# RViMLab/ECCV2022-multi-scale-and-cross-scale-contrastive-segmentation

Hardware: NVIDIA B200
Metric: ms+cs contrastive loss fwd+bwd anchor-pairs/s (higher is better)
Workload: dtype bf16

## Files before the change

eccv2022-multi-scale-and-cross-scale-contrastive-segmentation_b200/csrc/common.cuh:

```cuda
#pragma once
#include <cuda_runtime.h>
#include <cuda_bf16.h>
#include <cuda_fp16.h>
#include <stdint.h>
#include <stdio.h>
#include <stdarg.h>

#include "../../include/mscs.h"

namespace mscs {

void set_error(const char* fmt, ...);
const char* get_error();

#define MSCS_CHECK_ARG(cond, ...)                                   \
  do {                                                              \
    if (!(cond)) { ::mscs::set_error(__VA_ARGS__); return -1; }     \
  } while (0)

#define MSCS_CUDA(expr)                                                                   \
  do {                                                                                    \
    cudaError_t _e = (expr);                                                              \
    if (_e != cudaSuccess) {                                                              \
      ::mscs::set_error("%s failed: %s (%s:%d)", #expr, cudaGetErrorString(_e), __FILE__, \
                        __LINE__);                                                        \
      return (int)_e;                                                                     \
    }                                                                                     \
  } while (0)

#define MSCS_LAUNCH_CHECK()                                                               \
  do {                                                                                    \
    cudaError_t _e = cudaGetLastError();                                                  \
    if (_e != cudaSuccess) {                                                              \
      ::mscs::set_error("kernel launch failed: %s (%s:%d)", cudaGetErrorString(_e),       \
                        __FILE__, __LINE__);                                              \
      return (int)_e;                                                                     \
    }                                                                                     \
  } while (0)

static inline size_t align_up(size_t v, size_t a) { return (v + a - 1) / a * a; }
static inline int ceil_div(int a, int b) { return (a + b - 1) / b; }

bool pdl_enabled();

__device__ __forceinline__ void pdl_trigger() { asm volatile("griddepcontrol.launch_dependents;" ::: "memory"); }
__device__ __forceinline__ void pdl_wait() { asm volatile("griddepcontrol.wait;" ::: "memory"); }

template <typename... P, typename... A>
static inline cudaError_t launch_k(void (*kernel)(P...), dim3 grid, dim3 block, size_t smem, cudaStream_t st, A&&... args) {
  cudaLaunchConfig_t cfg{};
  cfg.gridDim = grid; cfg.blockDim = block; cfg.dynamicSmemBytes = smem; cfg.stream = st;
  cudaLaunchAttribute at{};
  at.id = cudaLaunchAttributeProgrammaticStreamSerialization;
  at.val.programmaticStreamSerializationAllowed = 1;
  cfg.attrs = &at;
  cfg.numAttrs = pdl_enabled() ? 1 : 0;
  return cudaLaunchKernelEx(&cfg, kernel, static_cast<P>(args)...);
}

__device__ __forceinline__ float warp_sum(float v) {
#pragma unroll
  for (int o = 16; o > 0; o >>= 1) v += __shfl_xor_sync(0xffffffffu, v, o);
  return v;
}

__device__ __forceinline__ float to_f32(float x) { return x; }
__device__ __forceinline__ float to_f32(__nv_bfloat16 x) { return __bfloat162float(x); }
__device__ __forceinline__ float to_f32(__half x) { return __half2float(x); }
template <typename T> __device__ __forceinline__ T from_f32(float x);
template <> __device__ __forceinline__ float from_f32<float>(float x) { return x; }
template <> __device__ __forceinline__ __nv_bfloat16 from_f32<__nv_bfloat16>(float x) { return __float2bfloat16_rn(x); }
template <> __device__ __forceinline__ __half from_f32<__half>(float x) { return __float2half_rn(x); }

__device__ __forceinline__ uint32_t pack2(__nv_bfloat16*, float a, float b) {
  const __nv_bfloat162 h = __floats2bfloat162_rn(a, b);
  return reinterpret_cast<const uint32_t&>(h);
}
__device__ __forceinline__ uint32_t pack2(__half*, float a, float b) {
  const __half2 h = __floats2half2_rn(a, b);
  return reinterpret_cast<const uint32_t&>(h);
}

__device__ __forceinline__ void st16_cs(float* p, const float (&v)[4]) {
  __stcs(reinterpret_cast<float4*>(p), make_float4(v[0], v[1], v[2], v[3]));
}
template <typename T>
__device__ __forceinline__ void st16_cs(T* p, const float (&v)[8]) {
  const uint4 u = make_uint4(pack2(p, v[0], v[1]), pack2(p, v[2], v[3]), pack2(p, v[4], v[5]), pack2(p, v[6], v[7]));
  __stcs(reinterpret_cast<uint4*>(p), u);
}

__device__ __forceinline__ void ld4(const float* p, float (&v)[4]) {
  const float4 x = *reinterpret_cast<const float4*>(p);
  v[0] = x.x; v[1] = x.y; v[2] = x.z; v[3] = x.w;
}
template <typename T>
__device__ __forceinline__ void ld4(const T* p, float (&v)[4]) {
  const uint2 u = *reinterpret_cast<const uint2*>(p);
  const T* h = reinterpret_cast<const T*>(&u);
#pragma unroll
  for (int q = 0; q < 4; ++q) v[q] = to_f32(h[q]);
}
__device__ __forceinline__ void st4_cs(float* p, const float (&v)[4]) { st16_cs(p, v); }
template <typename T>
__device__ __forceinline__ void st4_cs(T* p, const float (&v)[4]) {
  __stcs(reinterpret_cast<uint2*>(p), make_uint2(pack2(p, v[0], v[1]), pack2(p, v[2], v[3])));
}

static inline int dtype_bytes(int dtype) {
  return dtype == MSCS_DTYPE_F32 ? 4 : (dtype == MSCS_DTYPE_BF16 || dtype == MSCS_DTYPE_F16) ? 2 : 0;
}
// ... 3 lines not shown
```

eccv2022-multi-scale-and-cross-scale-contrastive-segmentation_b200/csrc/ptx.cuh:

```cuda
#pragma once
#include <cuda.h>
#include <cuda_runtime.h>
#include <stdint.h>

namespace mscs {
namespace ptx {

__device__ __forceinline__ uint32_t smem_u32(const void* p) {
  return static_cast<uint32_t>(__cvta_generic_to_shared(p));
}

__device__ __forceinline__ bool elect_one() {
  uint32_t pred;
  asm volatile(
      "{\n\t.reg .pred P;\n\t"
      "elect.sync _|P, 0xffffffff;\n\t"
      "selp.b32 %0, 1, 0, P;\n\t}"
      : "=r"(pred));
  return pred != 0;
}

__device__ __forceinline__ void mbar_init(uint64_t* bar, uint32_t count) {
  asm volatile("mbarrier.init.shared::cta.b64 [%0], %1;" ::"r"(smem_u32(bar)), "r"(count) : "memory");
}
// ... 179 lines not shown
  d |= (uint64_t)((sbo_bytes >> 4) & 0x3FFFu) << 32;
  d |= (uint64_t)1 << 46;
  d |= (uint64_t)2 << 61;
  return d;
}
__host__ __device__ constexpr uint32_t umma_idesc_bf16(int M, int N, int a_mn_major, int b_mn_major) {
  return (1u << 4) | (1u << 7) | (1u << 10) | ((uint32_t)a_mn_major << 15) | ((uint32_t)b_mn_major << 16) |
         ((uint32_t)(N >> 3) << 17) | ((uint32_t)(M >> 4) << 24);
}
__device__ __forceinline__ void umma_ss(uint32_t d_tmem, uint64_t a_desc, uint64_t b_desc, uint32_t idesc,
                                        uint32_t accumulate) {
  asm volatile(
      "{\n\t.reg .pred p;\n\t"
      "setp.ne.b32 p, %4, 0;\n\t"
      "tcgen05.mma.cta_group::1.kind::f16 [%0], %1, %2, %3, p;\n\t}"
      ::"r"(d_tmem), "l"(a_desc), "l"(b_desc), "r"(idesc), "r"(accumulate)
      : "memory");
}
__device__ __forceinline__ void umma_ts(uint32_t d_tmem, uint32_t a_tmem, uint64_t b_desc, uint32_t idesc,
                                        uint32_t accumulate) {
  asm volatile(
      "{\n\t.reg .pred p;\n\t"
      "setp.ne.b32 p, %4, 0;\n\t"
      "tcgen05.mma.cta_group::1.kind::f16 [%0], [%1], %2, %3, p;\n\t}"
      ::"r"(d_tmem), "r"(a_tmem), "l"(b_desc), "r"(idesc), "r"(accumulate)
      : "memory");
}
__device__ __forceinline__ void umma_ts2(uint32_t d_tmem, uint32_t a_tmem, uint32_t b_lo, uint32_t b_hi, uint32_t idesc,
                                         uint32_t accumulate) {
  asm volatile(
      "{\n\t.reg .pred p;\n\t.reg .b64 bd;\n\t"
      "setp.ne.b32 p, %5, 0;\n\t"
      "mov.b64 bd, {%2, %3};\n\t"
      "tcgen05.mma.cta_group::1.kind::f16 [%0], [%1], bd, %4, p;\n\t}"
      ::"r"(d_tmem), "r"(a_tmem), "r"(b_lo), "r"(b_hi), "r"(idesc), "r"(accumulate)
      : "memory");
}
__device__ __forceinline__ void umma_ss2(uint32_t d_tmem, uint32_t a_lo, uint32_t a_hi, uint32_t b_lo, uint32_t b_hi,
                                         uint32_t idesc, uint32_t accumulate) {
  asm volatile(
      "{\n\t.reg .pred p;\n\t.reg .b64 ad, bd;\n\t"
      "setp.ne.b32 p, %6, 0;\n\t"
      "mov.b64 ad, {%1, %2};\n\t"
      "mov.b64 bd, {%3, %4};\n\t"
      "tcgen05.mma.cta_group::1.kind::f16 [%0], ad, bd, %5, p;\n\t}"
      ::"r"(d_tmem), "r"(a_lo), "r"(a_hi), "r"(b_lo), "r"(b_hi), "r"(idesc), "r"(accumulate)
      : "memory");
}
__device__ __forceinline__ void umma_commit(uint64_t* bar) {
  asm volatile("tcgen05.commit.cta_group::1.mbarrier::arrive::one.shared::cluster.b64 [%0];" ::"r"(smem_u32(bar))
               : "memory");
}

__device__ __forceinline__ float ex2(float x) {
  float y;
  asm("ex2.approx.ftz.f32 %0, %1;" : "=f"(y) : "f"(x));
  return y;
}
__device__ __forceinline__ float ex2_poly(float v, float scale) {
  const float magic = 12582912.f;
  const float t = fmaf(v, scale, magic);
  const float n = t - magic;
  const float f = fmaf(v, scale, -n);
  float p = fmaf(0.009570100344717503f, f, 0.05591785907745361f);
  p = fmaf(p, f, 0.240247443318367f);
  p = fmaf(p, f, 0.6931217908859253f);
  p = fmaf(p, f, 0.9999992847442627f);
  return __int_as_float(__float_as_int(p) + (__float_as_int(t) << 23));
}
__device__ __forceinline__ uint64_t pack2(float lo, float hi) {
  uint64_t r;
  asm("mov.b64 %0, {%1, %2};" : "=l"(r) : "f"(lo), "f"(hi));
  return r;
}
__device__ __forceinline__ uint64_t pack2u(uint32_t lo, uint32_t hi) {
  uint64_t r;
  asm("mov.b64 %0, {%1, %2};" : "=l"(r) : "r"(lo), "r"(hi));
  return r;
}
__device__ __forceinline__ void unpack2(uint64_t v, float& lo, float& hi) {
  asm("mov.b64 {%0, %1}, %2;" : "=f"(lo), "=f"(hi) : "l"(v));
}
__device__ __forceinline__ uint64_t fma2(uint64_t a, uint64_t b, uint64_t c) {
  uint64_t d;
  asm("fma.rn.f32x2 %0, %1, %2, %3;" : "=l"(d) : "l"(a), "l"(b), "l"(c));
  return d;
}
__device__ __forceinline__ uint64_t mul2(uint64_t a, uint64_t b) {
  uint64_t d;
  asm("mul.rn.f32x2 %0, %1, %2;" : "=l"(d) : "l"(a), "l"(b));
  return d;
}
__device__ __forceinline__ uint64_t add2(uint64_t a, uint64_t b) {
  uint64_t d;
  asm("add.rn.f32x2 %0, %1, %2;" : "=l"(d) : "l"(a), "l"(b));
  return d;
}
__device__ __forceinline__ uint64_t ex2_poly2(uint64_t v, uint64_t scale2) {
  const uint64_t magic = pack2(12582912.f, 12582912.f), nmagic = pack2(-12582912.f, -12582912.f);
  const uint64_t t = fma2(v, scale2, magic);
  const uint64_t n = add2(t, nmagic);
  const uint64_t nn = n ^ 0x8000000080000000ull;
  const uint64_t f = fma2(v, scale2, nn);
  uint64_t p = fma2(pack2(0.009570100344717503f, 0.009570100344717503f), f, pack2(0.05591785907745361f, 0.05591785907745361f));
  p = fma2(p, f, pack2(0.240247443318367f, 0.240247443318367f));
  p = fma2(p, f, pack2(0.6931217908859253f, 0.6931217908859253f));
// ... 18 lines not shown
```

eccv2022-multi-scale-and-cross-scale-contrastive-segmentation_b200/csrc/sim_bwd.cu:

```cuda
#include "sim_tc.cuh"
#include <stdlib.h>

namespace mscs {

constexpr int kBwdEpiWarps = 16;
constexpr int kBwdThreads = 128 + 32 * kBwdEpiWarps;
constexpr int kBwdStages = 3;
constexpr int kBwdSub = 64;
constexpr uint32_t kTmX = 256, kTmS = 384;

struct BwdDev {
  const int* row_cls; const int* col_seg;
  const float* row_cs; const float* row_cpn; const float* row_neg;
  const float* col_cs; const float* col_cpn; const float* col_neg;
  const __nv_bfloat16* x_rows;
  float* dF; int ld;
  int n_rows, n_cols, self_mask, y_map;
  float scale_log2, out_scale;
};
struct BwdArgs {
  alignas(64) CUtensorMap maps[MSCS_MAX_SCALES];
  BwdDev p[MSCS_MAX_PASSES];
  WorkTable work;
  const float* grad_out;
  const int* rows_dev[MSCS_MAX_PASSES]; const int* cols_dev[MSCS_MAX_PASSES];
};

__host__ __device__ constexpr size_t bwd_smem_bytes(int KB) {
  return 1024 + (size_t)(kBwdStages * KB) * kBlkBytes + (size_t)kBwdEpiWarps * 2 * 3 * 32 * sizeof(float) + 256;
}

__device__ __forceinline__ uint32_t pack_bf16(float lo, float hi) {
  __nv_bfloat162 v = __floats2bfloat162_rn(lo, hi);
  return *reinterpret_cast<uint32_t*>(&v);
}
__device__ __forceinline__ void red_add_v4(float* addr, float a, float b, float c, float d) {
  asm volatile("red.global.add.v4.f32 [%0], {%1, %2, %3, %4};" ::"l"(addr), "f"(a), "f"(b), "f"(c), "f"(d)
               : "memory");
}

template <int KB, bool DEV>
__global__ void __launch_bounds__(kBwdThreads, 1) k_sim_bwd(const __grid_constant__ BwdArgs args) {
  constexpr int CP = KB * 64;
  extern __shared__ uint8_t smem_raw[];
  uint8_t* smem = reinterpret_cast<uint8_t*>((reinterpret_cast<uintptr_t>(smem_raw) + 1023) & ~uintptr_t(1023));
  uint8_t* smB = smem;
  float* cstat = reinterpret_cast<float*>(smB + (size_t)kBwdStages * KB * kBlkBytes);
  uint64_t* bars = reinterpret_cast<uint64_t*>(cstat + kBwdEpiWarps * 2 * 3 * 32);
  uint64_t* b_full = bars;
  uint64_t* b_empty = bars + 12;
  uint64_t* s_full = bars + 15;
  uint64_t* w_full = bars + 17;
  uint64_t* df_full = bars + 19;  uint64_t* df_empty = bars + 20;
  uint64_t* x_full = bars + 21;
  uint32_t* tmem_slot = reinterpret_cast<uint32_t*>(bars + 22);

  const int warp = threadIdx.x >> 5, lane = threadIdx.x & 31;
  pdl_trigger();
  if (warp == 0 && lane == 0) {
    for (int i = 0; i < kBwdStages; ++i) {
      ptx::mbar_init(&b_full[i], 1);
      ptx::mbar_init(&b_empty[i], 1);
    }
    for (int i = 0; i < 2; ++i) { ptx::mbar_init(&s_full[i], 1); ptx::mbar_init(&w_full[i], kBwdEpiWarps); }
    ptx::mbar_init(df_full, 1); ptx::mbar_init(df_empty, kBwdEpiWarps);
    ptx::mbar_init(x_full, kBwdEpiWarps);
    ptx::fence_barrier_init();
  }
  if (warp == 2) ptx::tmem_alloc(tmem_slot, 512);
  ptx::tc_fence_before();
  __syncthreads();
  ptx::tc_fence_after();
  const uint32_t tmem_base = *tmem_slot;
  pdl_wait();
#if defined(MSCS_WAIT_PROFILE) || defined(MSCS_TRACE)
  const unsigned long long prof_t0 = ptx::globaltimer_ns();
  const long long prof_c0 = clock64();
  (void)prof_t0;
// ... 214 lines not shown
          if (lane == 0) ptx::mbar_arrive(&w_full[sb]);
          MSCS_TRACE_EV(1 + ((warp - 4) >> 3), (warp - 4) & 7, t2);
        }
        publish_cols((un & 1) ^ 1);
      }
      if (warp == 4) MSCS_TRACE_EV(3, 0, 64u + seg);
      if (have_n && cq < KB)
        asm volatile("prefetch.global.L2 [%0];" ::"l"(args.p[nx.owner].x_rows + (size_t)(nx.rb * 128 + r_loc) * CP + cq * 64));
      ptx::mbar_wait(df_full, seg & 1, 222);
      ptx::tc_fence_after();
      if (warp == 4) MSCS_TRACE_EV(3, 1, 64u + seg);
      const float sc = p.out_scale * gout;
      float* drow = p.dF + (size_t)row * p.ld;
#pragma unroll 1
      for (int c0 = cq * (CP / 4); c0 < (cq + 1) * (CP / 4); c0 += 16) {
        uint32_t uu[16];
        ptx::tmem_ld16(tmem_dF + lane_base + c0, uu);
        ptx::tmem_ld_wait16(uu);
        if (valid) {
#pragma unroll
          for (int c = 0; c < 16; c += 4)
            red_add_v4(drow + c0 + c, __uint_as_float(uu[c]) * sc, __uint_as_float(uu[c + 1]) * sc,
                       __uint_as_float(uu[c + 2]) * sc, __uint_as_float(uu[c + 3]) * sc);
        }
      }
      ptx::tc_fence_before();
      __syncwarp();
      if (lane == 0) ptx::mbar_arrive(df_empty);
      if (warp == 4) MSCS_TRACE_EV(3, 2, 64u + seg);
      ++seg;
      sg = nx; have = have_n;
    }
  }
  __syncwarp();
  ptx::tc_fence_before();
  __syncthreads();
  if (warp == 2) ptx::tmem_dealloc(tmem_base, 512);
#ifdef MSCS_TRACE
  if (blockIdx.x == 5 && threadIdx.x == 0) ptx::g_trace[3 * 2048 + 255 * 8 + 6] = (unsigned long long)clock64();
  if (threadIdx.x == 0 && blockIdx.x < 256) {
    ptx::g_trace[3 * 2048 + 1024 + blockIdx.x] = (unsigned long long)(clock64() - prof_c0);
    ptx::g_trace[3 * 2048 + 1280 + blockIdx.x] = prof_t0;
    ptx::g_trace[3 * 2048 + 1536 + blockIdx.x] = ptx::globaltimer_ns();
  }
#endif
#ifdef MSCS_WAIT_PROFILE
  if (blockIdx.x == 0 && threadIdx.x == 0) {
    atomicAdd(&ptx::g_wait_ns[31], ptx::globaltimer_ns() - prof_t0);
    atomicAdd(&ptx::g_wait_cnt[31], (unsigned long long)(clock64() - prof_c0));
  }
#endif
}

}

using namespace mscs;

template <int KB, bool DEV>
static int launch_bwd(const BwdArgs& args, cudaStream_t st) {
  const size_t smem = bwd_smem_bytes(KB);
  if (int rc = ensure_trap_buffer()) return rc;
  MSCS_CUDA(cudaFuncSetAttribute(k_sim_bwd<KB, DEV>, cudaFuncAttributeMaxDynamicSharedMemorySize, (int)smem));
  MSCS_CUDA(launch_k(k_sim_bwd<KB, DEV>, persistent_ctas(), kBwdThreads, smem, st, args));
  MSCS_LAUNCH_CHECK();
  return 0;
}

extern "C" int mscs_sim_backward(const mscs_sim_job* job, const float* grad_out, float* const* dF_sets,
                                 const int32_t* dF_ld, void* stream_) {
  return mscs_sim_backward_sets(job, grad_out, dF_sets, dF_ld, 0xffffffffu, stream_);
}

extern "C" int mscs_sim_backward_sets(const mscs_sim_job* job, const float* grad_out, float* const* dF_sets,
                                      const int32_t* dF_ld, uint32_t set_mask, void* stream_) {
  int rc = validate_job(job);
  if (rc) return rc;
  MSCS_CHECK_ARG(job->work && grad_out && dF_sets && dF_ld, "null pointer argument");
  const bool dev_counts = job->terms[0].n1_dev != nullptr;
  for (int t = 0; t < job->num_terms; ++t)
    MSCS_CHECK_ARG((job->terms[t].n1_dev != nullptr) == dev_counts && (job->terms[t].n2_dev != nullptr) == dev_counts,
                   "term %d: n1_dev / n2_dev must be set for every term or for none", t);
  cudaStream_t st = (cudaStream_t)stream_;
  BwdPass passes[MSCS_MAX_PASSES];
  int np = build_passes(job, passes);
  {
    int kept = 0;
    for (int i = 0; i < np; ++i)
      if ((set_mask >> passes[i].row_set) & 1u) passes[kept++] = passes[i];
    np = kept;
    if (np == 0) return 0;
  }
  size_t fwd_items = 0, ranges = 0;
  for (int t = 0; t < job->num_terms; ++t) {
    fwd_items += (size_t)ceil_div(job->terms[t].N2, 256);
    ranges += align_up(sizeof(int2) * (size_t)job->terms[t].N1, 64) +
              align_up(sizeof(int2) * (size_t)ceil_div(job->terms[t].N1, 128) * 4, 64);
  }
  char* w = (char*)job->work + 4096 + ranges +
            2 * (align_up(sizeof(WorkItem) * fwd_items, 64) + align_up(sizeof(int) * (fwd_items + 1), 64));
  BwdArgs args{};
  args.grad_out = grad_out;
  const void* bases[MSCS_MAX_SCALES]; int nmaps = 0;
  auto map_of = [&](const void* base, int rows) -> int {
    for (int i = 0; i < nmaps; ++i) if (bases[i] == base) return i;
    if (nmaps == MSCS_MAX_SCALES) return -1;
    if (make_tensor_map(&args.maps[nmaps], base, (rows + 255) / 256 * 256, job->C_pad)) return -2;
    bases[nmaps] = base;
    return nmaps++;
  };
  BuildArgs b{};
  int nitems = 0;
  for (int i = 0; i < np; ++i) {
    const BwdPass& p = passes[i];
    const int ym = map_of(p.y_bf16, p.n_cols);
    if (ym == -2) return -1;
    MSCS_CHECK_ARG(ym >= 0, "too many distinct operand matrices");
    MSCS_CHECK_ARG(dF_sets[p.row_set] && dF_ld[p.row_set] >= job->C_pad && dF_ld[p.row_set] % 4 == 0,
                   "pass %d: dF buffer of set %d missing or leading dimension < C_pad", i, p.row_set);
    args.p[i] = BwdDev{p.row_cls, p.col_seg, p.row_cs, p.row_cpn, p.row_neg, p.col_cs, p.col_cpn, p.col_neg,
                       (const __nv_bfloat16*)p.x_bf16, dF_sets[p.row_set], dF_ld[p.row_set], p.n_rows, p.n_cols,
                       p.self_mask, ym, p.scale_log2, p.out_scale};
    b.t[i] = BuildTerm{p.row_cls, p.col_seg, p.n_rows, p.n_cols, nitems, p.rb_lo, 0, 1 << 30, p.n_rows_dev, p.n_cols_dev};
    args.rows_dev[i] = p.n_rows_dev; args.cols_dev[i] = p.n_cols_dev;
    nitems += p.rb_hi - p.rb_lo;
  }
  b.num_terms = np; b.nitems = nitems; b.rows_per_item = 128; b.mode = 0;
  b.pad = 6;
  static const int pad_env = [] { const char* e = getenv("MSCS_BWD_PAD"); return e ? atoi(e) : -1; }();
  if (pad_env >= 0) b.pad = pad_env;
  b.items = (WorkItem*)w; w += align_up(sizeof(WorkItem) * (size_t)nitems, 64);
  b.prefix = (int*)w;
  rc = launch_build_work(b, st);
  if (rc) return rc;
  args.work = WorkTable{b.items, b.prefix, nitems, b.pad};
  if (dev_counts) {
    switch (job->C_pad / 64) {
      case 1: return launch_bwd<1, true>(args, st);
      case 2: return launch_bwd<2, true>(args, st);
      case 3: return launch_bwd<3, true>(args, st);
      default: return launch_bwd<4, true>(args, st);
    }
  }
  switch (job->C_pad / 64) {
    case 1: return launch_bwd<1, false>(args, st);
    case 2: return launch_bwd<2, false>(args, st);
    case 3: return launch_bwd<3, false>(args, st);
    default: return launch_bwd<4, false>(args, st);
  }
}

extern "C" int mscs_debug_wait_profile_bwd(unsigned long long* ns_out, unsigned long long* cnt_out) {
  MSCS_CUDA(cudaDeviceSynchronize());
  MSCS_CUDA(cudaMemcpyFromSymbol(ns_out, ptx::g_wait_ns, sizeof(unsigned long long) * 32));
  MSCS_CUDA(cudaMemcpyFromSymbol(cnt_out, ptx::g_wait_cnt, sizeof(unsigned long long) * 32));
  unsigned long long zero[32] = {};
  MSCS_CUDA(cudaMemcpyToSymbol(ptx::g_wait_ns, zero, sizeof(zero)));
  MSCS_CUDA(cudaMemcpyToSymbol(ptx::g_wait_cnt, zero, sizeof(zero)));
  return 0;
}

extern "C" int mscs_debug_trace_bwd(unsigned long long* out, int max_events) {
#ifdef MSCS_TRACE
  MSCS_CUDA(cudaDeviceSynchronize());
  const int n = max_events < 8192 ? max_events : 8192;
  MSCS_CUDA(cudaMemcpyFromSymbol(out, ptx::g_trace, sizeof(unsigned long long) * n));
  static unsigned long long zeros[8192];
  MSCS_CUDA(cudaMemcpyToSymbol(ptx::g_trace, zeros, sizeof(zeros)));
  return n;
#else
  (void)out; (void)max_events;
  return 0;
#endif
}
```

eccv2022-multi-scale-and-cross-scale-contrastive-segmentation_b200/csrc/sim_fwd.cu:

```cuda
#include "sim_tc.cuh"
#include <stdlib.h>
#ifdef MSCS_TRACE
#ifndef MSCS_TRACE_MODE
#define MSCS_TRACE_MODE 0
#endif
#undef MSCS_TRACE_EV
#define MSCS_TRACE_EV(slot, k, tile)                                                                 \
  do {                                                                                               \
    if (MODE == MSCS_TRACE_MODE && blockIdx.x == 5 && (threadIdx.x & 31) == 0 && (tile) < 256u)                    \
      mscs::ptx::g_trace[(slot) * 2048 + (tile) * 8 + (k)] = (unsigned long long)clock64();          \
  } while (0)
#endif

namespace mscs {

constexpr int kFwdKeys = 256;
constexpr int kFwdEpiWarps = 16;
constexpr int kFwdThreads = 128 + 32 * kFwdEpiWarps;
constexpr int kFwdColsPerThread = kFwdKeys / 2;
constexpr int kFwdStages = 5;
constexpr int kAccBars = 2;

struct FwdTerm {
  const int* a_cls; const int* k_seg;
// ... 333 lines not shown
  __shared__ int wsum[32];
  pdl_trigger();
  pdl_wait();
  const int mode = a.mode + (int)blockIdx.x;
  WorkItem* const items = blockIdx.x ? a.items1 : a.items;
  int* const prefix = blockIdx.x ? a.prefix1 : a.prefix;
  if (threadIdx.x == 0) { carry = 0; prefix[0] = 0; }
  __syncthreads();
  for (int base = 0; base < a.nitems; base += blockDim.x) {
    const int i = base + threadIdx.x;
    int len = 0;
    if (i < a.nitems) {
      int ti = 0;
      for (int q = 1; q < a.num_terms; ++q) if (i >= a.t[q].item_base) ti = q;
      const BuildTerm& t = a.t[ti];
      const int rb = t.blk_lo + i - t.item_base;
      const int tN1 = t.n1_dev ? *t.n1_dev : t.N1, tN2 = t.n2_dev ? *t.n2_dev : t.N2;
      int ct0 = 0, ct1 = (tN2 + kTileN - 1) / kTileN;
      if (rb * a.rows_per_item >= tN1) {
        ct0 = ct1 = 0;
      } else if (mode == 1) {
        const int r0 = rb * a.rows_per_item, r1 = min(tN1, r0 + a.rows_per_item) - 1;
        const int p0 = t.k_seg[t.a_cls[r0]], p1 = t.k_seg[t.a_cls[r1] + 1];
        if (p1 > p0) { ct0 = p0 / kTileN; ct1 = (p1 + kTileN - 1) / kTileN; } else { ct0 = ct1 = 0; }
      }
      ct0 = max(ct0, t.ct_lo); ct1 = max(ct0, min(ct1, t.ct_hi));
      items[i] = WorkItem{ti, rb, ct0, ct1};
      len = ct1 > ct0 ? ct1 - ct0 + a.pad : 0;
    }
    int s = len;
#pragma unroll
    for (int o = 1; o < 32; o <<= 1) { int v = __shfl_up_sync(0xffffffffu, s, o); if ((threadIdx.x & 31) >= o) s += v; }
    if ((threadIdx.x & 31) == 31) wsum[threadIdx.x >> 5] = s;
    __syncthreads();
    if (threadIdx.x < 32) {
      int w = wsum[threadIdx.x], ws = w;
#pragma unroll
      for (int o = 1; o < 32; o <<= 1) { int v = __shfl_up_sync(0xffffffffu, ws, o); if ((int)threadIdx.x >= o) ws += v; }
      wsum[threadIdx.x] = ws - w;
    }
    __syncthreads();
    const int incl = carry + wsum[threadIdx.x >> 5] + s;
    if (i < a.nitems) prefix[i + 1] = incl;
    __syncthreads();
    if (threadIdx.x == blockDim.x - 1) carry = incl;
    __syncthreads();
  }
}

typedef CUresult (*EncodeTiledFn)(CUtensorMap*, CUtensorMapDataType, cuuint32_t, void*, const cuuint64_t*,
                                  const cuuint64_t*, const cuuint32_t*, const cuuint32_t*, CUtensorMapInterleave,
                                  CUtensorMapSwizzle, CUtensorMapL2promotion, CUtensorMapFloatOOBfill);

int make_tensor_map(CUtensorMap* out, const void* base, int rows, int c_pad) {
  static EncodeTiledFn fn = nullptr;
  if (!fn) {
    void* p = nullptr;
    cudaDriverEntryPointQueryResult qr;
    MSCS_CUDA(cudaGetDriverEntryPoint("cuTensorMapEncodeTiled", &p, cudaEnableDefault, &qr));
    MSCS_CHECK_ARG(p != nullptr && qr == cudaDriverEntryPointSuccess, "cuTensorMapEncodeTiled not available");
    fn = (EncodeTiledFn)p;
  }
  cuuint64_t dims[2] = {(cuuint64_t)c_pad, (cuuint64_t)rows};
  cuuint64_t strides[1] = {(cuuint64_t)c_pad * 2};
  cuuint32_t box[2] = {(cuuint32_t)kKBlk, 128};
  cuuint32_t estr[2] = {1, 1};
  CUresult r = CUDA_SUCCESS;
  for (int attempt = 0; attempt < 2; ++attempt) {
    r = fn(out, CU_TENSOR_MAP_DATA_TYPE_BFLOAT16, 2, const_cast<void*>(base), dims, strides, box, estr,
           CU_TENSOR_MAP_INTERLEAVE_NONE, CU_TENSOR_MAP_SWIZZLE_128B, CU_TENSOR_MAP_L2_PROMOTION_L2_256B,
           CU_TENSOR_MAP_FLOAT_OOB_FILL_NONE);
    if (r != CUDA_ERROR_INVALID_CONTEXT) break;
    MSCS_CUDA(cudaFree(nullptr));
  }
  MSCS_CHECK_ARG(r == CUDA_SUCCESS, "cuTensorMapEncodeTiled failed with CUresult %d", (int)r);
  return 0;
}

int launch_build_work(const BuildArgs& b, cudaStream_t st) {
  MSCS_CUDA(launch_k(k_build_work, b.items1 ? 2 : 1, 1024, 0, st, b));
  MSCS_LAUNCH_CHECK();
  return 0;
}

int sm_count() {
  static int n = 0;
  if (!n) { int dev = 0; cudaGetDevice(&dev); cudaDeviceGetAttribute(&n, cudaDevAttrMultiProcessorCount, dev); }
  return n > 0 ? n : 148;
}

int persistent_ctas() {
  static const int spare = [] { const char* e = getenv("MSCS_SPARE_SMS"); const int v = e ? atoi(e) : 1; return v < 0 ? 0 : v; }();
  const int n = sm_count() - spare;
  return n > 0 ? n : 1;
}

struct FwdTuning { int pad; bool timeline; };
static const FwdTuning& fwd_tuning() {
  static const FwdTuning t = [] {
    FwdTuning v{0, false};
    if (const char* e = getenv("MSCS_FWD_PAD")) v.pad = atoi(e);
    v.timeline = getenv("MSCS_FWD_TIMELINE") != nullptr;
    return v;
  }();
  return t;
}

template <int KB, int MODE>
static int launch_fwd_k(const FwdArgs& args, cudaStream_t st) {
  const size_t smem = fwd_smem_bytes(KB);
  static bool attr_done = false;
  if (!attr_done) {
    MSCS_CUDA(cudaFuncSetAttribute(k_sim_fwd<KB, MODE>, cudaFuncAttributeMaxDynamicSharedMemorySize, (int)smem));
    attr_done = true;
  }
  MSCS_CUDA(launch_k(k_sim_fwd<KB, MODE>, persistent_ctas(), kFwdThreads, smem, st, args));
  MSCS_LAUNCH_CHECK();
  return 0;
// ... 156 lines not shown
```

eccv2022-multi-scale-and-cross-scale-contrastive-segmentation_b200/csrc/sim_tc.cuh:

```cuda
#pragma once
#include "ptx.cuh"
#include "sim_common.cuh"

namespace mscs {

constexpr int kTileN = 128;
constexpr int kKBlk = 64;
constexpr int kBlkBytes = 128 * 128;

struct WorkItem { int owner, rb, ct0, ct1; };
struct WorkTable { const WorkItem* items; const int* prefix; int nitems; int pad; };

struct Segment { int owner, rb, c_begin, c_end; };

struct Walker {
  const WorkTable& w;
  int u, u_end, item;
  __device__ Walker(const WorkTable& wt) : w(wt) {
    const long long total = wt.prefix[wt.nitems];
    u = (int)(total * blockIdx.x / gridDim.x);
    u_end = (int)(total * (blockIdx.x + 1) / gridDim.x);
    int lo = 0, hi = wt.nitems;
    while (lo < hi) {
      int mid = (lo + hi + 1) >> 1;
      if (wt.prefix[mid] <= u) lo = mid; else hi = mid - 1;
    }
    item = lo;
  }
  __device__ bool next(Segment& s) {
    while (u < u_end) {
      while (w.prefix[item + 1] <= u) ++item;
      const WorkItem it = w.items[item];
      const int base = w.prefix[item];
      const int e = min(u_end, w.prefix[item + 1]);
      const int b0 = max(0, u - base - w.pad), b1 = max(0, e - base - w.pad);
      u = e;
      if (b1 > b0) {
        s.owner = it.owner; s.rb = it.rb;
        s.c_begin = it.ct0 + b0;
        s.c_end = it.ct0 + b1;
        return true;
      }
    }
    return false;
  }
};

struct BuildTerm { const int* a_cls; const int* k_seg; int N1, N2, item_base, blk_lo, ct_lo, ct_hi;
                   const int* n1_dev; const int* n2_dev; };
struct BuildArgs { BuildTerm t[MSCS_MAX_PASSES]; int num_terms, nitems, rows_per_item, mode, pad; WorkItem* items; int* prefix;
                   WorkItem* items1; int* prefix1; };
int launch_build_work(const BuildArgs& b, cudaStream_t st);
int trap_buffer_device_ptr(unsigned long long** out);
static inline int ensure_trap_buffer() {
  static bool done = false;
  if (done) return 0;
  unsigned long long* d = nullptr;
  if (int rc = trap_buffer_device_ptr(&d)) return rc;
  MSCS_CUDA(cudaMemcpyToSymbol(ptx::g_trap_buf, &d, sizeof(d)));
  done = true;
  return 0;
}
int sm_count();
int persistent_ctas();

int make_tensor_map(CUtensorMap* out, const void* base, int rows, int c_pad);

}
```

Measured before the change: 452.5 billion.

## Add 2-CTA cluster backward kernel with paired tcgen05 MMA for C_pad 256

Adds a clustered backward kernel for the C_pad=256 case. Two CTAs cooperate on 256-row blocks using cta_group::2 tcgen05 MMAs, paired TMA loads and multicast commits. The X tile stays resident in shared memory per segment, and the dF accumulation for all 256 channels happens in TMEM. The work table is rebuilt at 256 rows per item, and the single-CTA path's KB=4 template is dropped. The aim is to halve per-CTA operand traffic and raise MMA efficiency with larger M tiles, at the cost of cluster synchronisation, fewer launched clusters and more complex barrier logic.

```diff
diff --git a/eccv2022-multi-scale-and-cross-scale-contrastive-segmentation_b200/csrc/common.cuh b/eccv2022-multi-scale-and-cross-scale-contrastive-segmentation_b200/csrc/common.cuh
--- a/eccv2022-multi-scale-and-cross-scale-contrastive-segmentation_b200/csrc/common.cuh
+++ b/eccv2022-multi-scale-and-cross-scale-contrastive-segmentation_b200/csrc/common.cuh
@@ -57,6 +57,20 @@
   cfg.numAttrs = pdl_enabled() ? 1 : 0;
   return cudaLaunchKernelEx(&cfg, kernel, static_cast<P>(args)...);
 }
+template <typename... P, typename... A>
+static inline cudaError_t launch_k_cluster(void (*kernel)(P...), int cluster_x, dim3 grid, dim3 block, size_t smem,
+                                           cudaStream_t st, A&&... args) {
+  cudaLaunchConfig_t cfg{};
+  cfg.gridDim = grid; cfg.blockDim = block; cfg.dynamicSmemBytes = smem; cfg.stream = st;
+  cudaLaunchAttribute at[2]{};
+  at[0].id = cudaLaunchAttributeClusterDimension;
+  at[0].val.clusterDim.x = cluster_x; at[0].val.clusterDim.y = 1; at[0].val.clusterDim.z = 1;
+  at[1].id = cudaLaunchAttributeProgrammaticStreamSerialization;
+  at[1].val.programmaticStreamSerializationAllowed = 1;
+  cfg.attrs = at;
+  cfg.numAttrs = pdl_enabled() ? 2 : 1;
+  return cudaLaunchKernelEx(&cfg, kernel, static_cast<P>(args)...);
+}
 
 __device__ __forceinline__ float warp_sum(float v) {
 #pragma unroll
diff --git a/eccv2022-multi-scale-and-cross-scale-contrastive-segmentation_b200/csrc/ptx.cuh b/eccv2022-multi-scale-and-cross-scale-contrastive-segmentation_b200/csrc/ptx.cuh
--- a/eccv2022-multi-scale-and-cross-scale-contrastive-segmentation_b200/csrc/ptx.cuh
+++ b/eccv2022-multi-scale-and-cross-scale-contrastive-segmentation_b200/csrc/ptx.cuh
@@ -255,6 +255,75 @@
                : "memory");
 }
 
+__device__ __forceinline__ uint32_t cluster_ctarank() {
+  uint32_t r;
+  asm volatile("mov.u32 %0, %%cluster_ctarank;" : "=r"(r));
+  return r;
+}
+__device__ __forceinline__ uint32_t cluster_id_x() {
+  uint32_t r;
+  asm volatile("mov.u32 %0, %%clusterid.x;" : "=r"(r));
+  return r;
+}
+__device__ __forceinline__ uint32_t nclusters_x() {
+  uint32_t r;
+  asm volatile("mov.u32 %0, %%nclusterid.x;" : "=r"(r));
+  return r;
+}
+__device__ __forceinline__ void cluster_arrive() { asm volatile("barrier.cluster.arrive.release.aligned;" ::: "memory"); }
+__device__ __forceinline__ void cluster_wait() { asm volatile("barrier.cluster.wait.acquire.aligned;" ::: "memory"); }
+__device__ __forceinline__ void cluster_sync() { cluster_arrive(); cluster_wait(); }
+__device__ __forceinline__ uint32_t mapa(const void* p, uint32_t rank) {
+  uint32_t r;
+  asm volatile("mapa.shared::cluster.u32 %0, %1, %2;" : "=r"(r) : "r"(smem_u32(p)), "r"(rank));
+  return r;
+}
+__device__ __forceinline__ void mbar_arrive_cluster(uint32_t bar_cluster) {
+  asm volatile("mbarrier.arrive.release.cluster.shared::cluster.b64 _, [%0];" ::"r"(bar_cluster) : "memory");
+}
+__device__ __forceinline__ void tma_load_2d_pair(void* smem_dst, const CUtensorMap* m, uint32_t bar_cluster, int x, int y) {
+  asm volatile(
+      "cp.async.bulk.tensor.2d.cta_group::2.shared::cluster.global.mbarrier::complete_tx::bytes [%0], [%1, {%3, %4}], [%2];"
+      ::"r"(smem_u32(smem_dst)), "l"(reinterpret_cast<uint64_t>(m)), "r"(bar_cluster), "r"(x), "r"(y)
+      : "memory");
+}
+__device__ __forceinline__ void tmem_alloc_pair(uint32_t* smem_out, uint32_t ncols) {
+  asm volatile("tcgen05.alloc.cta_group::2.sync.aligned.shared::cta.b32 [%0], %1;" ::"r"(smem_u32(smem_out)),
+               "r"(ncols)
+               : "memory");
+  asm volatile("tcgen05.relinquish_alloc_permit.cta_group::2.sync.aligned;" ::: "memory");
+}
+__device__ __forceinline__ void tmem_dealloc_pair(uint32_t taddr, uint32_t ncols) {
+  asm volatile("tcgen05.dealloc.cta_group::2.sync.aligned.b32 %0, %1;" ::"r"(taddr), "r"(ncols) : "memory");
+}
+__device__ __forceinline__ void umma_ss2_pair(uint32_t d_tmem, uint32_t a_lo, uint32_t a_hi, uint32_t b_lo, uint32_t b_hi,
+                                              uint32_t idesc, uint32_t accumulate) {
+  asm volatile(
+      "{\n\t.reg .pred p;\n\t.reg .b64 ad, bd;\n\t"
+      "setp.ne.b32 p, %6, 0;\n\t"
+      "mov.b64 ad, {%1, %2};\n\t"
+      "mov.b64 bd, {%3, %4};\n\t"
+      "tcgen05.mma.cta_group::2.kind::f16 [%0], ad, bd, %5, p;\n\t}"
+      ::"r"(d_tmem), "r"(a_lo), "r"(a_hi), "r"(b_lo), "r"(b_hi), "r"(idesc), "r"(accumulate)
+      : "memory");
+}
+__device__ __forceinline__ void umma_ts2_pair(uint32_t d_tmem, uint32_t a_tmem, uint32_t b_lo, uint32_t b_hi,
+                                              uint32_t idesc, uint32_t accumulate) {
+  asm volatile(
+      "{\n\t.reg .pred p;\n\t.reg .b64 bd;\n\t"
+      "setp.ne.b32 p, %5, 0;\n\t"
+      "mov.b64 bd, {%2, %3};\n\t"
+      "tcgen05.mma.cta_group::2.kind::f16 [%0], [%1], bd, %4, p;\n\t}"
+      ::"r"(d_tmem), "r"(a_tmem), "r"(b_lo), "r"(b_hi), "r"(idesc), "r"(accumulate)
+      : "memory");
+}
+__device__ __forceinline__ void umma_commit_pair(uint64_t* bar, uint16_t cta_mask) {
+  asm volatile(
+      "tcgen05.commit.cta_group::2.mbarrier::arrive::one.shared::cluster.multicast::cluster.b64 [%0], %1;"
+      ::"r"(smem_u32(bar)), "h"(cta_mask)
+      : "memory");
+}
+
 __device__ __forceinline__ float ex2(float x) {
   float y;
   asm("ex2.approx.ftz.f32 %0, %1;" : "=f"(y) : "f"(x));
diff --git a/eccv2022-multi-scale-and-cross-scale-contrastive-segmentation_b200/csrc/sim_bwd.cu b/eccv2022-multi-scale-and-cross-scale-contrastive-segmentation_b200/csrc/sim_bwd.cu
--- a/eccv2022-multi-scale-and-cross-scale-contrastive-segmentation_b200/csrc/sim_bwd.cu
+++ b/eccv2022-multi-scale-and-cross-scale-contrastive-segmentation_b200/csrc/sim_bwd.cu
@@ -24,6 +24,7 @@
   WorkTable work;
   const float* grad_out;
   const int* rows_dev[MSCS_MAX_PASSES]; const int* cols_dev[MSCS_MAX_PASSES];
+  int x_map[MSCS_MAX_PASSES]; int row_lo[MSCS_MAX_PASSES], row_hi[MSCS_MAX_PASSES];
 };
 
 __host__ __device__ constexpr size_t bwd_smem_bytes(int KB) {
@@ -344,6 +345,286 @@
 #endif
 }
 
+constexpr int kPairSStages = 3, kPairDStages = 2;
+constexpr uint32_t kPairTmS = 256;
+constexpr int kPairPartBytes = 4 * kBlkBytes / 2;
+__host__ __device__ constexpr size_t bwd_pair_smem_bytes() {
+  return 1024 + 4 * (size_t)kBlkBytes + (size_t)(kPairSStages + kPairDStages) * kPairPartBytes + 256;
+}
+
+template <bool DEV>
+__global__ void __launch_bounds__(kBwdThreads, 1) k_sim_bwd_pair(const __grid_constant__ BwdArgs args) {
+  constexpr int CP = 256;
+  extern __shared__ uint8_t smem_raw[];
+  uint8_t* smem = reinterpret_cast<uint8_t*>((reinterpret_cast<uintptr_t>(smem_raw) + 1023) & ~uintptr_t(1023));
+  uint8_t* smX = smem;
+  uint8_t* smS = smX + 4 * kBlkBytes;
+  uint8_t* smD = smS + kPairSStages * kPairPartBytes;
+  uint64_t* bars = reinterpret_cast<uint64_t*>(smD + kPairDStages * kPairPartBytes);
+  uint64_t* s_full = bars;        uint64_t* s_empty = bars + 3;   uint64_t* d_full = bars + 6;   uint64_t* d_empty = bars + 8;
+  uint64_t* acc_full = bars + 10; uint64_t* w_full = bars + 12;   uint64_t* x_full = bars + 14;  uint64_t* x_empty = bars + 15;
+  uint64_t* df_full = bars + 16;  uint64_t* df_empty = bars + 17;
+  uint32_t* tmem_slot = reinterpret_cast<uint32_t*>(bars + 18);
+
+  const int warp = threadIdx.x >> 5, lane = threadIdx.x & 31;
+  const uint32_t rank = ptx::cluster_ctarank();
+  const bool leader = rank == 0;
+  pdl_trigger();
+  if (warp == 0 && lane == 0) {
+    for (int i = 0; i < kPairSStages; ++i) { ptx::mbar_init(&s_full[i], 1); ptx::mbar_init(&s_empty[i], 1); }
+    for (int i = 0; i < 2; ++i) {
+      ptx::mbar_init(&d_full[i], 1); ptx::mbar_init(&d_empty[i], 1);
+      ptx::mbar_init(&acc_full[i], 1); ptx::mbar_init(&w_full[i], 2 * kBwdEpiWarps);
+    }
+    ptx::mbar_init(x_full, 1); ptx::mbar_init(x_empty, 1);
+    ptx::mbar_init(df_full, 1); ptx::mbar_init(df_empty, 2 * kBwdEpiWarps);
+    ptx::fence_barrier_init();
+  }
+  if (warp == 2) ptx::tmem_alloc_pair(tmem_slot, 512);
+  ptx::tc_fence_before();
+  ptx::cluster_sync();
+  ptx::tc_fence_after();
+  const uint32_t tmem_base = *tmem_slot;
+  pdl_wait();
+  const int cl = (int)ptx::cluster_id_x(), ncl = (int)ptx::nclusters_x();
+
+  if (warp == 0 || warp == 3) {
+    const bool dpart = warp == 3;
+    Walker wk(args.work, cl, ncl);
+    Segment sg;
+    uint32_t u = 0, seg = 0;
+    while (wk.next(sg)) {
+      const BwdDev& p = args.p[sg.owner];
+      const CUtensorMap* ym = &args.maps[p.y_map];
+      if (!dpart) {
+        ptx::mbar_wait(x_empty, (seg & 1) ^ 1, 232);
+        if (ptx::elect_one()) {
+          if (leader) ptx::mbar_expect_tx(x_full, 2 * 4 * kBlkBytes);
+          const uint32_t xb = ptx::mapa(x_full, 0);
+          const int r0 = sg.rb * 256 + (int)rank * 128;
+          for (int kb = 0; kb < 4; ++kb)
+            for (int h = 0; h < 2; ++h)
+              ptx::tma_load_2d_pair(smX + kb * kBlkBytes + h * (kBlkBytes / 2), &args.maps[args.x_map[sg.owner]], xb,
+                                    kb * kKBlk, r0 + 64 * h);
+        }
+        __syncwarp();
+      }
+      for (int ct = sg.c_begin; ct < sg.c_end; ++ct, ++u) {
+        const uint32_t nst = dpart ? kPairDStages : kPairSStages, st = u % nst, ph = (u / nst) & 1;
+        uint64_t* full = dpart ? &d_full[st] : &s_full[st];
+        ptx::mbar_wait(dpart ? &d_empty[st] : &s_empty[st], ph ^ 1, dpart ? 231 : 230);
+        if (ptx::elect_one()) {
+          if (leader) ptx::mbar_expect_tx(full, 2 * kPairPartBytes);
+          const uint32_t fb = ptx::mapa(full, 0);
+          if (dpart) {
+            for (int j = 0; j < 2; ++j)
+              for (int h = 0; h < 2; ++h)
+                ptx::tma_load_2d_pair(smD + st * kPairPartBytes + j * kBlkBytes + h * (kBlkBytes / 2), ym, fb,
+                                      (2 * (int)rank + j) * kKBlk, ct * kTileN + 64 * h);
+          } else {
+            for (int kb = 0; kb < 4; ++kb)
+              ptx::tma_load_2d_pair(smS + st * kPairPartBytes + kb * (kBlkBytes / 2), ym, fb, kb * kKBlk,
+                                    ct * kTileN + 64 * (int)rank);
+          }
+        }
+        __syncwarp();
+      }
+      ++seg;
+    }
+  } else if (warp == 1) {
+    if (leader) {
+      constexpr uint32_t idesc_s = ptx::umma_idesc_bf16(256, kTileN, 0, 0);
+      constexpr uint32_t idesc_d = ptx::umma_idesc_bf16(256, CP, 0, 1);
+      const uint64_t xdesc = ptx::umma_desc_sw128(ptx::smem_u32(smX), 16, 1024);
+      const uint64_t sdesc = ptx::umma_desc_sw128(ptx::smem_u32(smS), 16, 1024);
+      const uint64_t ddesc = ptx::umma_desc_sw128(ptx::smem_u32(smD), kBlkBytes, 1024);
+      const uint32_t x_lo = (uint32_t)xdesc, x_hi = (uint32_t)(xdesc >> 32);
+      const uint32_t s_lo = (uint32_t)sdesc, s_hi = (uint32_t)(sdesc >> 32);
+      const uint32_t d_lo = (uint32_t)ddesc, d_hi = (uint32_t)(ddesc >> 32);
+      Walker wk(args.work, cl, ncl);
+      Segment sg;
+      uint32_t u = 0, seg = 0;
+      auto emit_s = [&](uint32_t t_, bool last) {
+        const uint32_t sb_ = t_ & 1, st_ = t_ % kPairSStages;
+#pragma unroll
+        for (int kk = 0; kk < 16; ++kk)
+          ptx::umma_ss2_pair(tmem_base + kPairTmS + sb_ * kTileN, x_lo + (((kk >> 2) * kBlkBytes + (kk & 3) * 32) >> 4),
+                             x_hi, s_lo + ((st_ * kPairPartBytes + (kk >> 2) * (kBlkBytes / 2) + (kk & 3) * 32) >> 4),
+                             s_hi, idesc_s, kk != 0);
+        ptx::umma_commit_pair(&acc_full[sb_], 3);
+        ptx::umma_commit_pair(&s_empty[st_], 3);
+        if (last) ptx::umma_commit_pair(x_empty, 3);
+      };
+      auto emit_d = [&](uint32_t t_, uint32_t first) {
+        const uint32_t sb_ = t_ & 1;
+        const uint32_t w_tm = tmem_base + kPairTmS + sb_ * kTileN;
+#pragma unroll
+        for (int i = 0; i < 8; ++i)
+          ptx::umma_ts2_pair(tmem_base, w_tm + (i >> 1) * 32 + (i & 1) * 8,
+                             d_lo + ((sb_ * kPairPartBytes + i * 16 * 128) >> 4), d_hi, idesc_d, (first != 0) | (i != 0));
+        ptx::umma_commit_pair(&d_empty[sb_], 3);
+      };
+      while (wk.next(sg)) {
+        const uint32_t ntiles = (uint32_t)(sg.c_end - sg.c_begin);
+        ptx::mbar_wait(x_full, seg & 1, 242);
+        ptx::mbar_wait(&s_full[u % kPairSStages], (u / kPairSStages) & 1, 240);
+        ptx::tc_fence_after();
+        if (ptx::elect_one()) emit_s(u, ntiles == 1);
+        __syncwarp();
+        ptx::mbar_wait(df_empty, (seg & 1) ^ 1, 243);
+        for (uint32_t j = 0; j < ntiles; ++j) {
+          const uint32_t cur = u + j;
+          if (ptx::elect_one()) {
+            if (j + 1 < ntiles) {
+              ptx::mbar_wait(&s_full[(cur + 1) % kPairSStages], ((cur + 1) / kPairSStages) & 1, 240);
+              ptx::tc_fence_after();
+              emit_s(cur + 1, j + 2 == ntiles);
+            }
+            ptx::mbar_wait(&d_full[cur & 1], (cur >> 1) & 1, 241);
+            ptx::mbar_spin_wait(&w_full[cur & 1], (cur >> 1) & 1, 244);
+            ptx::tc_fence_after();
+            emit_d(cur, j);
+          }
+          __syncwarp();
+        }
+        if (ptx::elect_one()) ptx::umma_commit_pair(df_full, 3);
+        __syncwarp();
+        u += ntiles; ++seg;
+      }
+    }
+  } else if (warp >= 4) {
+    const int cq = (warp - 4) >> 2, quad = warp & 3;
+    const int r_loc = quad * 32 + lane;
+    const uint32_t lane_base = (uint32_t)(quad * 32) << 16;
+    const float gout = *args.grad_out;
+    Walker wk(args.work, cl, ncl);
+    Segment sg, nx;
+    uint32_t t = 0, seg = 0;
+    bool have = wk.next(sg);
+    while (have) {
+      const bool have_n = wk.next(nx);
+      const BwdDev& p = args.p[sg.owner];
+      const int row = sg.rb * 256 + (int)rank * 128 + r_loc;
+      int dev_rows = 0, dev_cols = 0;
+      if constexpr (DEV) { dev_rows = *args.rows_dev[sg.owner]; dev_cols = *args.cols_dev[sg.owner]; }
+      const bool valid = row < (DEV ? dev_rows : p.n_rows) && row >= args.row_lo[sg.owner] && row < args.row_hi[sg.owner];
+      int p0 = 0, p1 = 0;
+      if (valid) { const int y = p.row_cls[row]; p0 = p.col_seg[y]; p1 = p.col_seg[y + 1]; }
+      const unsigned plen = (unsigned)(p1 - p0);
+      int wmin = valid ? p0 : 0x7fffffff, wmax = valid ? p1 : 0;
+#pragma unroll
+      for (int o = 16; o > 0; o >>= 1) {
+        wmin = min(wmin, __shfl_xor_sync(0xffffffffu, wmin, o));
+        wmax = max(wmax, __shfl_xor_sync(0xffffffffu, wmax, o));
+      }
+      const float rcs = (valid && p.row_cs) ? p.row_cs[row] : 0.f;
+      const float rcpn = (valid && p.row_cpn) ? p.row_cpn[row] : 0.f;
+      const float rneg = (valid && p.row_neg) ? p.row_neg[row] : 1.f;
+      const int self_col = p.self_mask ? row : -1;
+      const float scale = p.scale_log2;
+      const uint64_t scale2 = ptx::pack2(scale, scale), rcs2 = ptx::pack2(rcs, rcs);
+      float pf_s = 0.f, pf_pn = 0.f, pf_neg = 1.f;
+      auto prefetch_cols = [&](int ct_) {
+        pf_s = 0.f; pf_pn = 0.f; pf_neg = 1.f;
+        if (ct_ < sg.c_end) {
+          const int c = ct_ * kTileN + cq * 32 + lane;
+          if (c < (DEV ? dev_cols : p.n_cols)) {
+            if (p.col_cs) pf_s = p.col_cs[c];
+            if (p.col_cpn) pf_pn = p.col_cpn[c];
+            if (p.col_neg) pf_neg = p.col_neg[c];
+          }
+        }
+      };
+      prefetch_cols(sg.c_begin);
+      for (int ct = sg.c_begin; ct < sg.c_end; ++ct, ++t) {
+        const uint32_t sb = t & 1;
+        const float cl_s = pf_s, cl_pn = pf_pn, cl_neg = pf_neg;
+        prefetch_cols(ct + 1);
+        const int cb0 = ct * kTileN + cq * 32;
+        ptx::mbar_wait(&acc_full[sb], (t >> 1) & 1, 251);
+        ptx::tc_fence_after();
+        const uint32_t taddr = tmem_base + lane_base + kPairTmS + sb * kTileN + cq * 32;
+#pragma unroll
+        for (int hh = 0; hh < 2; ++hh) {
+          const int cb = cb0 + hh * 16;
+          const bool touches = !(cb + 16 <= wmin || cb >= wmax);
+          uint32_t v[16];
+          ptx::tmem_ld16(taddr + hh * 16, v);
+          ptx::tmem_ld_wait16(v);
+          uint32_t packed[8];
+          if (!touches) {
+#pragma unroll
+            for (int c = 0; c < 16; c += 4) {
+              const int l0 = hh * 16 + c;
+              const float4 cc = make_float4(__shfl_sync(0xffffffffu, cl_s, l0), __shfl_sync(0xffffffffu, cl_s, l0 + 1),
+                                            __shfl_sync(0xffffffffu, cl_s, l0 + 2), __shfl_sync(0xffffffffu, cl_s, l0 + 3));
+#pragma unroll
+              for (int q = 0; q < 2; ++q) {
+                float x0, x1;
+                ptx::unpack2(ptx::mul2(ptx::pack2u(v[c + 2 * q], v[c + 2 * q + 1]), scale2), x0, x1);
+                const uint64_t e2 = ptx::pack2(ptx::ex2(x0), ptx::ex2(x1));
+                const uint64_t c2 = ptx::add2(rcs2, q == 0 ? ptx::pack2(cc.x, cc.y) : ptx::pack2(cc.z, cc.w));
+                float w0, w1;
+                ptx::unpack2(ptx::mul2(e2, c2), w0, w1);
+                packed[(c >> 1) + q] = pack_bf16(w0, w1);
+              }
+            }
+          } else {
+#pragma unroll
+            for (int c = 0; c < 16; c += 2) {
+              float w[2];
+#pragma unroll
+              for (int q = 0; q < 2; ++q) {
+                const int j = c + q;
+                const int col = cb + j;
+                const float e = ptx::ex2(__uint_as_float(v[j]) * scale);
+                const bool ispos = (unsigned)(col - p0) < plen;
+                const float cs_j = __shfl_sync(0xffffffffu, cl_s, hh * 16 + j);
+                const float cpn_j = __shfl_sync(0xffffffffu, cl_pn, hh * 16 + j);
+                const float cneg_j = __shfl_sync(0xffffffffu, cl_neg, hh * 16 + j);
+                const float wn = e * (rcs + cs_j);
+                const float wp = -(rcpn * ptx::rcp(e + rneg) + cpn_j * ptx::rcp(e + cneg_j));
+                w[q] = ispos ? (col == self_col ? 0.f : wp) : wn;
+              }
+              packed[c >> 1] = pack_bf16(w[0], w[1]);
+            }
+          }
+          ptx::tmem_st8(taddr + hh * 8, packed);
+        }
+        ptx::tmem_st_wait();
+        ptx::tc_fence_before();
+        __syncwarp();
+        if (lane == 0) ptx::mbar_arrive_cluster(ptx::mapa(&w_full[sb], 0));
+      }
+      ptx::mbar_wait(df_full, seg & 1, 252);
+      ptx::tc_fence_after();
+      const float sc = p.out_scale * gout;
+      float* drow = p.dF + (size_t)row * p.ld;
+#pragma unroll 1
+      for (int c0 = cq * (CP / 4); c0 < (cq + 1) * (CP / 4); c0 += 16) {
+        uint32_t uu[16];
+        ptx::tmem_ld16(tmem_base + lane_base + c0, uu);
+        ptx::tmem_ld_wait16(uu);
+        if (valid) {
+#pragma unroll
+          for (int c = 0; c < 16; c += 4)
+            red_add_v4(drow + c0 + c, __uint_as_float(uu[c]) * sc, __uint_as_float(uu[c + 1]) * sc,
+                       __uint_as_float(uu[c + 2]) * sc, __uint_as_float(uu[c + 3]) * sc);
+        }
+      }
+      ptx::tc_fence_before();
+      __syncwarp();
+      if (lane == 0) ptx::mbar_arrive_cluster(ptx::mapa(df_empty, 0));
+      ++seg;
+      sg = nx; have = have_n;
+    }
+  }
+  __syncwarp();
+  ptx::tc_fence_before();
+  ptx::cluster_sync();
+  if (warp == 2) ptx::tmem_dealloc_pair(tmem_base, 512);
+}
+
 }
 
 using namespace mscs;
@@ -354,6 +635,32 @@
   if (int rc = ensure_trap_buffer()) return rc;
   MSCS_CUDA(cudaFuncSetAttribute(k_sim_bwd<KB, DEV>, cudaFuncAttributeMaxDynamicSharedMemorySize, (int)smem));
   MSCS_CUDA(launch_k(k_sim_bwd<KB, DEV>, persistent_ctas(), kBwdThreads, smem, st, args));
+  MSCS_LAUNCH_CHECK();
+  return 0;
+}
+
+template <bool DEV>
+static int launch_bwd_pair(const BwdArgs& args, cudaStream_t st) {
+  const size_t smem = bwd_pair_smem_bytes();
+  if (int rc = ensure_trap_buffer()) return rc;
+  MSCS_CUDA(cudaFuncSetAttribute(k_sim_bwd_pair<DEV>, cudaFuncAttributeMaxDynamicSharedMemorySize, (int)smem));
+  static int clusters = 0;
+  if (!clusters) {
+    cudaLaunchConfig_t cfg{};
+    cfg.gridDim = dim3(2 * (sm_count() / 2)); cfg.blockDim = kBwdThreads; cfg.dynamicSmemBytes = smem;
+    cudaLaunchAttribute at{};
+    at.id = cudaLaunchAttributeClusterDimension;
+    at.val.clusterDim.x = 2; at.val.clusterDim.y = 1; at.val.clusterDim.z = 1;
+    cfg.attrs = &at; cfg.numAttrs = 1;
+    int active = 0;
+    MSCS_CUDA(cudaOccupancyMaxActiveClusters(&active, k_sim_bwd_pair<DEV>, &cfg));
+    const int spare = sm_count() - persistent_ctas();
+    int n = active - (spare + 1) / 2;
+    if (n > persistent_ctas() / 2) n = persistent_ctas() / 2;
+    MSCS_CHECK_ARG(n >= 1, "no CTA pair of the backward kernel fits on this device (%d co-resident)", active);
+    clusters = n;
+  }
+  MSCS_CUDA(launch_k_cluster(k_sim_bwd_pair<DEV>, 2, 2 * clusters, kBwdThreads, smem, st, args));
   MSCS_LAUNCH_CHECK();
   return 0;
 }
@@ -390,13 +697,15 @@
   }
   char* w = (char*)job->work + 4096 + ranges +
             2 * (align_up(sizeof(WorkItem) * fwd_items, 64) + align_up(sizeof(int) * (fwd_items + 1), 64));
+  const bool pair = job->C_pad == 256;
+  const int rows_per_item = pair ? 256 : 128;
   BwdArgs args{};
   args.grad_out = grad_out;
   const void* bases[MSCS_MAX_SCALES]; int nmaps = 0;
   auto map_of = [&](const void* base, int rows) -> int {
     for (int i = 0; i < nmaps; ++i) if (bases[i] == base) return i;
     if (nmaps == MSCS_MAX_SCALES) return -1;
-    if (make_tensor_map(&args.maps[nmaps], base, (rows + 255) / 256 * 256, job->C_pad)) return -2;
+    if (make_tensor_map(&args.maps[nmaps], base, (rows + 255) / 256 * 256, job->C_pad, pair ? 64 : 128)) return -2;
     bases[nmaps] = base;
     return nmaps++;
   };
@@ -405,18 +714,21 @@
   for (int i = 0; i < np; ++i) {
     const BwdPass& p = passes[i];
     const int ym = map_of(p.y_bf16, p.n_cols);
-    if (ym == -2) return -1;
-    MSCS_CHECK_ARG(ym >= 0, "too many distinct operand matrices");
+    const int xm = pair ? map_of(p.x_bf16, p.n_rows) : 0;
+    if (ym == -2 || xm == -2) return -1;
+    MSCS_CHECK_ARG(ym >= 0 && xm >= 0, "too many distinct operand matrices");
     MSCS_CHECK_ARG(dF_sets[p.row_set] && dF_ld[p.row_set] >= job->C_pad && dF_ld[p.row_set] % 4 == 0,
                    "pass %d: dF buffer of set %d missing or leading dimension < C_pad", i, p.row_set);
     args.p[i] = BwdDev{p.row_cls, p.col_seg, p.row_cs, p.row_cpn, p.row_neg, p.col_cs, p.col_cpn, p.col_neg,
                        (const __nv_bfloat16*)p.x_bf16, dF_sets[p.row_set], dF_ld[p.row_set], p.n_rows, p.n_cols,
                        p.self_mask, ym, p.scale_log2, p.out_scale};
-    b.t[i] = BuildTerm{p.row_cls, p.col_seg, p.n_rows, p.n_cols, nitems, p.rb_lo, 0, 1 << 30, p.n_rows_dev, p.n_cols_dev};
+    const int blk_lo = p.rb_lo * 128 / rows_per_item, blk_hi = ceil_div(p.rb_hi * 128, rows_per_item);
+    b.t[i] = BuildTerm{p.row_cls, p.col_seg, p.n_rows, p.n_cols, nitems, blk_lo, 0, 1 << 30, p.n_rows_dev, p.n_cols_dev};
     args.rows_dev[i] = p.n_rows_dev; args.cols_dev[i] = p.n_cols_dev;
-    nitems += p.rb_hi - p.rb_lo;
-  }
-  b.num_terms = np; b.nitems = nitems; b.rows_per_item = 128; b.mode = 0;
+    args.x_map[i] = xm; args.row_lo[i] = p.rb_lo * 128; args.row_hi[i] = p.rb_hi * 128;
+    nitems += blk_hi - blk_lo;
+  }
+  b.num_terms = np; b.nitems = nitems; b.rows_per_item = rows_per_item; b.mode = 0;
   b.pad = 6;
   static const int pad_env = [] { const char* e = getenv("MSCS_BWD_PAD"); return e ? atoi(e) : -1; }();
   if (pad_env >= 0) b.pad = pad_env;
@@ -425,19 +737,18 @@
   rc = launch_build_work(b, st);
   if (rc) return rc;
   args.work = WorkTable{b.items, b.prefix, nitems, b.pad};
+  if (pair) return dev_counts ? launch_bwd_pair<true>(args, st) : launch_bwd_pair<false>(args, st);
   if (dev_counts) {
     switch (job->C_pad / 64) {
       case 1: return launch_bwd<1, true>(args, st);
       case 2: return launch_bwd<2, true>(args, st);
-      case 3: return launch_bwd<3, true>(args, st);
-      default: return launch_bwd<4, true>(args, st);
+      default: return launch_bwd<3, true>(args, st);
     }
   }
   switch (job->C_pad / 64) {
     case 1: return launch_bwd<1, false>(args, st);
     case 2: return launch_bwd<2, false>(args, st);
-    case 3: return launch_bwd<3, false>(args, st);
-    default: return launch_bwd<4, false>(args, st);
+    default: return launch_bwd<3, false>(args, st);
   }
 }
 
diff --git a/eccv2022-multi-scale-and-cross-scale-contrastive-segmentation_b200/csrc/sim_fwd.cu b/eccv2022-multi-scale-and-cross-scale-contrastive-segmentation_b200/csrc/sim_fwd.cu
--- a/eccv2022-multi-scale-and-cross-scale-contrastive-segmentation_b200/csrc/sim_fwd.cu
+++ b/eccv2022-multi-scale-and-cross-scale-contrastive-segmentation_b200/csrc/sim_fwd.cu
@@ -409,7 +409,7 @@
                                   const cuuint64_t*, const cuuint32_t*, const cuuint32_t*, CUtensorMapInterleave,
                                   CUtensorMapSwizzle, CUtensorMapL2promotion, CUtensorMapFloatOOBfill);
 
-int make_tensor_map(CUtensorMap* out, const void* base, int rows, int c_pad) {
+int make_tensor_map(CUtensorMap* out, const void* base, int rows, int c_pad, int box_rows) {
   static EncodeTiledFn fn = nullptr;
   if (!fn) {
     void* p = nullptr;
@@ -420,7 +420,7 @@
   }
   cuuint64_t dims[2] = {(cuuint64_t)c_pad, (cuuint64_t)rows};
   cuuint64_t strides[1] = {(cuuint64_t)c_pad * 2};
-  cuuint32_t box[2] = {(cuuint32_t)kKBlk, 128};
+  cuuint32_t box[2] = {(cuuint32_t)kKBlk, (cuuint32_t)box_rows};
   cuuint32_t estr[2] = {1, 1};
   CUresult r = CUDA_SUCCESS;
   for (int attempt = 0; attempt < 2; ++attempt) {
diff --git a/eccv2022-multi-scale-and-cross-scale-contrastive-segmentation_b200/csrc/sim_tc.cuh b/eccv2022-multi-scale-and-cross-scale-contrastive-segmentation_b200/csrc/sim_tc.cuh
--- a/eccv2022-multi-scale-and-cross-scale-contrastive-segmentation_b200/csrc/sim_tc.cuh
+++ b/eccv2022-multi-scale-and-cross-scale-contrastive-segmentation_b200/csrc/sim_tc.cuh
@@ -16,10 +16,11 @@
 struct Walker {
   const WorkTable& w;
   int u, u_end, item;
-  __device__ Walker(const WorkTable& wt) : w(wt) {
+  __device__ Walker(const WorkTable& wt) : Walker(wt, blockIdx.x, gridDim.x) {}
+  __device__ Walker(const WorkTable& wt, int part, int nparts) : w(wt) {
     const long long total = wt.prefix[wt.nitems];
-    u = (int)(total * blockIdx.x / gridDim.x);
-    u_end = (int)(total * (blockIdx.x + 1) / gridDim.x);
+    u = (int)(total * part / nparts);
+    u_end = (int)(total * (part + 1) / nparts);
     int lo = 0, hi = wt.nitems;
     while (lo < hi) {
       int mid = (lo + hi + 1) >> 1;
@@ -64,6 +65,6 @@
 int sm_count();
 int persistent_ctas();
 
-int make_tensor_map(CUtensorMap* out, const void* base, int rows, int c_pad);
+int make_tensor_map(CUtensorMap* out, const void* base, int rows, int c_pad, int box_rows = 128);
 
 }
```

Result: slower. 427.3 billion (median of 6 runs) (-5.6%).
